# boguszjelinski/taxidispatcher

Measured on AMD Instinct MI355X. Metric: NxN assignments/sec, higher is better.
Workload: dtype int32; 1 GPU; g1 N=16384: device cost write (4N^2 B) + exact assignment, total checked == optimum; n=16384, parallelism=single GPU

## Files before the change

taxidispatcher_amd/csrc/td_assign.hip:

```cpp
#include <dlfcn.h>
#include <limits.h>
#include <stdlib.h>

#include <type_traits>

#include "td_common.h"

using namespace td;

namespace {

template <typename CT>
struct Tr;
template <>
struct Tr<uint8_t> {
    using PT = int32_t;
    static constexpr int E = 16;
    static constexpr uint32_t SENT = 0xFFu;
    static constexpr int64_t LIMIT = 254;
    static constexpr int32_t BIG = 1 << 28;
    static constexpr int32_t KMAX = INT32_MAX;
};
template <>
struct Tr<uint16_t> {
// ... 130 lines not shown
int g_defer_const = 1;
int g_shape = 1;
int g_shape_max_n = 1 << 20;
int g_narrow_price = 1;
long long g_np_plimit = NP_PLIMIT;
int g_fuse_t = 2;
int g_fuse_spec = 1;
int g_fused_rounds = 8;
int g_fuse_gen = 1;
int g_tick_rounds = 5;
int g_forest = 1;
int g_forest_min_n = 2048;
long long g_forest_w0 = 16;
long long g_forest_wx = 16;
int g_blocks = -1;
int g_blocks_min_n = 12288;
int g_zs_rounds = 4;
int g_zs_sep = 0;
int g_hop_passes = 2;
int g_hop_max_rows = HOP_FMAX;
int g_lazy_cc = 1;
int g_hop_global = 1;
int g_one_trip = 1;
int g_zs_global_rounds = 6;
int g_core = 1;
int g_core_k = 64;
int g_core_min_n = 8192;
int g_core_mode = 1;
double g_core_eps = 1.0;
int g_rand_test = 1;
int g_rand_div = 8192;
int g_rand_rounds = 48;
int g_rand_repeat = 1;
double g_rand_corr = 0.12;
int g_core_patience = 6;
int g_solver_eps = 0;
int g_eps_theta = 8;
long long g_eps0_mult = 4;
void read_tunables()
{
    static bool done = false;
    if (done) return;
    done = true;
    if (const char *e = getenv("TD_MAX_ROUNDS")) g_max_rounds = std::max(1, std::min(48, atoi(e)));
    if (const char *e = getenv("TD_TIE_EVICT")) g_tie_evict = atoi(e) != 0;
    if (const char *e = getenv("TD_LDS_ROUNDS")) g_lds_rounds = std::max(0, atoi(e));
// ... 47 lines not shown
    if (const char *e = getenv("TD_LINE")) g_line = atoi(e) != 0;
    if (const char *e = getenv("TD_LINE_MIN_N")) g_line_min_n = std::max(2, atoi(e));
    if (const char *e = getenv("TD_PSAP8_GRID")) g_psap8_grid = std::max(1, std::min(192, atoi(e)));
    if (const char *e = getenv("TD_CORE")) g_core = atoi(e) != 0;
    if (const char *e = getenv("TD_CORE_K")) g_core_k = std::max(2, std::min(200, atoi(e)));
    if (const char *e = getenv("TD_CORE_MIN_N")) g_core_min_n = std::max(256, atoi(e));
    if (const char *e = getenv("TD_CORE_MODE")) g_core_mode = atoi(e);
    if (const char *e = getenv("TD_CORE_EPS")) g_core_eps = atof(e);
    if (const char *e = getenv("TD_CORE_PATIENCE")) g_core_patience = std::max(1, atoi(e));
    if (const char *e = getenv("TD_RAND_TEST")) g_rand_test = atoi(e) != 0;
    if (const char *e = getenv("TD_RAND_DIV")) g_rand_div = std::max(1, atoi(e));
    if (const char *e = getenv("TD_RAND_ROUNDS")) g_rand_rounds = std::max(1, std::min(48, atoi(e)));
    if (const char *e = getenv("TD_RAND_CORR")) g_rand_corr = atof(e);
    if (const char *e = getenv("TD_RAND_REPEAT")) g_rand_repeat = std::max(1, atoi(e));
    if (const char *e = getenv("TD_BLOCKS")) g_blocks = std::max(-1, std::min(HOP_BMAX, atoi(e)));
    if (const char *e = getenv("TD_BLOCKS_MIN_N")) g_blocks_min_n = std::max(0, atoi(e));
    if (const char *e = getenv("TD_ZS_ROUNDS")) g_zs_rounds = std::max(0, std::min(32, atoi(e)));
    if (const char *e = getenv("TD_ZS_SEP")) g_zs_sep = atoi(e) != 0;
    if (const char *e = getenv("TD_HOP_PASSES")) g_hop_passes = std::max(0, std::min(8, atoi(e)));
    if (const char *e = getenv("TD_HOP_MAX_ROWS")) g_hop_max_rows = std::max(1, atoi(e));
    if (const char *e = getenv("TD_HOP_GLOBAL")) g_hop_global = atoi(e) != 0;
    if (const char *e = getenv("TD_ONE_TRIP")) g_one_trip = atoi(e) != 0;
    if (const char *e = getenv("TD_LAZY_CC")) g_lazy_cc = atoi(e) != 0;
    if (const char *e = getenv("TD_ZS_GLOBAL_ROUNDS")) g_zs_global_rounds = std::max(1, std::min(48, atoi(e)));
}

template <typename CT>
__device__ __forceinline__ void unpack(const uint4 &v, uint32_t *out);
template <>
__device__ __forceinline__ void unpack<uint8_t>(const uint4 &v, uint32_t *o)
{
    const uint32_t w[4] = {v.x, v.y, v.z, v.w};
#pragma unroll
    for (int k = 0; k < 4; k++) {
        o[4 * k + 0] = w[k] & 0xFFu;
        o[4 * k + 1] = (w[k] >> 8) & 0xFFu;
        o[4 * k + 2] = (w[k] >> 16) & 0xFFu;
        o[4 * k + 3] = w[k] >> 24;
    }
}
template <>
__device__ __forceinline__ void unpack<u8e>(const uint4 &v, uint32_t *o)
{
    const uint32_t w[4] = {v.x, v.y, v.z, v.w};
    const uint32_t esc = g_esc8;
#pragma unroll
// ... 144 lines not shown
__global__ __launch_bounds__(256) void k_compress_rest(int n, int nrows, int row0, int nchunks, int rpb, const int32_t *__restrict__ cost,
                                                       uint8_t *__restrict__ cc, const int32_t *__restrict__ rowmin,
                                                       const int *__restrict__ ctl)
{
    if (ctl[CTL_FLAG]) return;
    const int nq = n >> 2, qpb = rpb >> 2;
    const size_t pitch = (size_t)nchunks * 16;
    for (int row = blockIdx.x; row < nrows; row += gridDim.x) {
        const int mn = rowmin[row];
        const int q0 = ((row0 + row) / rpb) * qpb;
        const int4 *s4 = reinterpret_cast<const int4 *>(cost + (int64_t)row * n);
        uint32_t *dst = reinterpret_cast<uint32_t *>(cc + (size_t)row * pitch);
        for (int q = threadIdx.x; q < nq; q += 256) {
            if ((unsigned)(q - q0) < (unsigned)qpb) continue;
            const int4 x4 = s4[q];
            const uint32_t a = (uint32_t)(x4.x - mn), b = (uint32_t)(x4.y - mn), c = (uint32_t)(x4.z - mn), d = (uint32_t)(x4.w - mn);
            dst[q] = (a & 0xFF) | ((b & 0xFF) << 8) | ((c & 0xFF) << 16) | (d << 24);
        }
    }
}

__device__ __forceinline__ void shape_decide(int n, int *__restrict__ ctl);

template <typename CT, int VPT, int THREADS, bool BID0 = false, int LH = 0>
__global__ __launch_bounds__(THREADS) void k_compress_reg(
    int n, int nrows, int nchunks, const int32_t *__restrict__ cost, CT *__restrict__ cc, int32_t *__restrict__ rowmin, int *__restrict__ ctl,
    int *__restrict__ rconst, const long long *__restrict__ skip, unsigned long long *__restrict__ bid = nullptr, int row0 = 0,
    int *__restrict__ r2c = nullptr ,
    int probe_tickets = 0 ,
    int zs_rpb = 0 ,
    int diag_only = 0 )
{
    static_assert(!BID0 || sizeof(CT) == 1, "round 0 out of the compress pass: 1-byte cells");
    if (skip && *skip) return;
    constexpr int E = Tr<CT>::E;
    constexpr int NW = THREADS / 64;
    __shared__ int s_mn[2][NW], s_mx[2][NW];
    __shared__ int s_fp[2][BID0 ? NW : 1], s_c0[2][BID0 ? NW : 1];
    const int tid = threadIdx.x, lane = tid & 63, w = tid >> 6;
    const size_t pitch = (size_t)nchunks * E;
    const int nq = n >> 2;
    int par = 0;
    int prev_row = -1, prev_rot = 0;
    long long wmax = 0;
    auto flush_bid = [&](int slot) {
        if constexpr (BID0) {
            if (prev_row < 0 || w != 0) return;
            int fp = INT_MAX, c0 = 0;
#pragma unroll
            for (int k = 0; k < NW; k++) {
// ... 14 lines not shown
                }
#pragma unroll
                for (int o = 32; o > 0; o >>= 1) m2 = min(m2, (unsigned)__shfl_xor((int)m2, o));
            }
            if (lane == 0) {
                const int grow = row0 + prev_row;
                const int t1 = fp / E;
                int ch = t1 + prev_rot;
                if (zs_rpb) {
                    const int zcpb = zs_rpb / E;
                    if (ch >= zcpb) ch -= zcpb;
                    ch += (grow / zs_rpb) * zcpb;
                } else if (ch >= nchunks)
                    ch -= nchunks;
                const int j1 = ch * E + (fp - t1 * E);
                const unsigned long long inc = (c0 >= 2 || m2 == 255) ? 0ull : (unsigned long long)m2;
                if (inc == 0 && (grow & 15) == 0) atomicAdd(&ctl[CTL_TIED], 1);
                if (j1 < n) atomicMax(&bid[j1], (inc << ROW_BITS) | (unsigned long long)(grow + 1));
            }
        }
    };
    constexpr int VR = VPT - LH;
    extern __shared__ int4 s_rowh[];
    for (int row = blockIdx.x; row < nrows; row += gridDim.x) {
        const int4 *s4 = reinterpret_cast<const int4 *>(cost + (int64_t)row * n);
        int4 v[VPT];
#pragma unroll
        for (int k = 0; k < VPT; k++) {
            const int q = k * THREADS + tid;
#if defined(TD_NT) && (TD_NT & 2)
            if (q < nq) {
                typedef int v4i __attribute__((ext_vector_type(4)));
                const v4i t4 = __builtin_nontemporal_load(reinterpret_cast<const v4i *>(s4) + q);
                v[k] = make_int4(t4.x, t4.y, t4.z, t4.w);
            }
#else
            if (q < nq) v[k] = s4[q];
#endif
        }
        int mn = INT_MAX, mx = INT_MIN;
#pragma unroll
        for (int k = 0; k < VPT; k++) {
            const int q = k * THREADS + tid;
            if (q < nq) {
                mn = min(min(mn, v[k].x), min(v[k].y, min(v[k].z, v[k].w)));
                mx = max(max(mx, v[k].x), max(v[k].y, max(v[k].z, v[k].w)));
            }
// ... 2410 lines not shown
            using PT = typename Tr<CT>::PT;
            const int npad = nchunks * E;
            const PT padkey = (PT)(Tr<CT>::BIG << 1) | (PT)1;
            const int gi = (std::max(npad, (int)CTL_WORDS) + 255) / 256;
            const int gc = nq <= 256 * 16 ? gb : std::max(1, std::min(nrows, c.n_cu * 2));
            tickets = sv.probe ? gi + gc : 0;
            uint8_t *ob_z = nullptr;
            if (g_one_trip && zs_rpb > 0) {
                if ((rc = ensure(sv.ob, (size_t)npad + 64))) return rc;
                ob_z = (uint8_t *)sv.ob.p;
            }
            unsigned long long *fin_z = g_one_trip ? (unsigned long long *)((char *)sv.misc.p + FIN_OFF) : nullptr;
            k_init_state<PT><<<gi, 256, 0, c.stream>>>(n, npad, nrows, (PT *)sv.price.p, padkey, (int *)sv.owner.p, (int *)sv.r2c.p,
                                                       (unsigned long long *)sv.bid.p, ctl, nullptr, sv.probe, tickets, ob_z, fin_z);
            if (!fin_z) TD_HIP(hipMemsetAsync((char *)sv.misc.p + FIN_OFF, 0, 16, c.stream));
            sv.ob_clear = ob_z != nullptr;
            sv.bid0_done = true;
        }
        ProfScope ps(TD_K_COMPRESS);
        unsigned long long *bidp = (unsigned long long *)sv.bid.p;
        int *defer_r2c = sv.defer_const ? (int *)sv.r2c.p : nullptr;
        if (g_creg && vec && nq <= 256 * 16) {
            const int g2 = std::max(1, std::min(nrows, c.n_cu * g_cgrid));
#define TD_CR(VPT) k_compress_reg<CT, VPT, 256><<<g2, 256, 0, c.stream>>>(n, nrows, nchunks, sv.d_cost, cc, rm, ctl, rcs, sv.skip)
            if (nq <= 256) { TD_CR(1); }
            else if (nq <= 512) { TD_CR(2); }
            else if (nq <= 1024) { TD_CR(4); }
            else if (nq <= 2048) { TD_CR(8); }
            else if (bid0_kernel) {
                if constexpr (sizeof(CT) == 1) {
                    static const int shape = getenv("TD_BID0_SHAPE") ? atoi(getenv("TD_BID0_SHAPE")) : 0;
                    if (shape == 1)
                        k_compress_reg<CT, 4, 1024, true><<<gb, 1024, 0, c.stream>>>(n, nrows, nchunks, sv.d_cost, cc, rm, ctl, rcs, sv.skip, bidp,
                                                                                    sv.row0, defer_r2c, tickets, zs_rpb, diag);
                    else
                        k_compress_reg<CT, 8, 512, true><<<gb, 512, 0, c.stream>>>(n, nrows, nchunks, sv.d_cost, cc, rm, ctl, rcs, sv.skip, bidp,
                                                                                   sv.row0, defer_r2c, tickets, zs_rpb, diag);
                    sv.zs_done = zs_rpb > 0;
                    sv.cc_partial = diag != 0;
                    sv.cc_rpb = zs_rpb;
                }
            } else {
                static const int cshape = getenv("TD_CREG_SHAPE") ? atoi(getenv("TD_CREG_SHAPE")) : 0;
                if (cshape == 1)
                    k_compress_reg<CT, 8, 512><<<gb, 512, 0, c.stream>>>(n, nrows, nchunks, sv.d_cost, cc, rm, ctl, rcs, sv.skip);
                else if (cshape == 2)
                    k_compress_reg<CT, 4, 1024><<<gb, 1024, 0, c.stream>>>(n, nrows, nchunks, sv.d_cost, cc, rm, ctl, rcs, sv.skip);
                else { TD_CR(16); }
            }
#undef TD_CR
        } else if (g_creg && vec && nq <= 1024 * 16) {
            const int g4 = std::max(1, std::min(nrows, c.n_cu * 2));
            static const int clds = getenv("TD_CLDS") ? atoi(getenv("TD_CLDS")) : 0;
            if (bid0_kernel) {
                if constexpr (sizeof(CT) == 1)
                {
                    if (clds == 8) {
                        const int shm = 8 * 1024 * 16;
                        (void)hipFuncSetAttribute((const void *)k_compress_reg<CT, 16, 1024, true, 8>, hipFuncAttributeMaxDynamicSharedMemorySize, shm);
                        k_compress_reg<CT, 16, 1024, true, 8><<<g4, 1024, shm, c.stream>>>(n, nrows, nchunks, sv.d_cost, cc, rm, ctl, rcs, sv.skip, bidp,
                                                                                          sv.row0, defer_r2c, tickets, zs_rpb, diag);
                    } else if (clds == 4) {
                        const int shm = 4 * 1024 * 16;
                        (void)hipFuncSetAttribute((const void *)k_compress_reg<CT, 16, 1024, true, 4>, hipFuncAttributeMaxDynamicSharedMemorySize, shm);
                        k_compress_reg<CT, 16, 1024, true, 4><<<g4, 1024, shm, c.stream>>>(n, nrows, nchunks, sv.d_cost, cc, rm, ctl, rcs, sv.skip, bidp,
                                                                                          sv.row0, defer_r2c, tickets, zs_rpb, diag);
                    } else
                        k_compress_reg<CT, 16, 1024, true><<<g4, 1024, 0, c.stream>>>(n, nrows, nchunks, sv.d_cost, cc, rm, ctl, rcs, sv.skip, bidp,
                                                                                      sv.row0, defer_r2c, tickets, zs_rpb, diag);
                    sv.zs_done = zs_rpb > 0;
                    sv.cc_partial = diag != 0;
                    sv.cc_rpb = zs_rpb;
                }
            } else
                k_compress_reg<CT, 16, 1024><<<g4, 1024, 0, c.stream>>>(n, nrows, nchunks, sv.d_cost, cc, rm, ctl, rcs, sv.skip);
        } else if (vec)
            k_compress<CT, true><<<grid, 256, 0, c.stream>>>(n, nrows, nchunks, sv.d_cost, cc, rm, ctl, rcs, sv.skip);
        else
            k_compress<CT, false><<<grid, 256, 0, c.stream>>>(n, nrows, nchunks, sv.d_cost, cc, rm, ctl, rcs, sv.skip);
    }
    TD_HIP(hipGetLastError());
    if (speculate) {
        *fits = true;
        sv.nconst = -1;
    } else {
        TD_HIP(hipMemcpyAsync(c.pinned, ctl, CTL_ALL * sizeof(int), hipMemcpyDeviceToHost, c.stream));
        TD_HIP(hipStreamSynchronize(c.stream));
        *fits = (((int *)c.pinned)[CTL_FLAG] == 0);
        sv.nconst = ((int *)c.pinned)[CTL_NCONST];
        sv.range_seen = (int64_t)(((const unsigned long long *)((int *)c.pinned + CTL_RSEEN))[0]);
        if (!*fits) c.stats[6] = (int64_t)(((const unsigned long long *)((int *)c.pinned + CTL_RANGE))[0]);
    }
    if (*fits) {
        sv.bpc = IsNP<CT>::value ? 5 : (int)sizeof(CT);
        sv.nchunks = nchunks;
        sv.npad = nchunks * E;
    }
    return TD_OK;
// ... 79 lines not shown
    *range = (int64_t)(((const unsigned long long *)(h + CTL_RANGE))[0]);
    *fits = h[CTL_FLAG] == 0 && *range <= (int64_t)Tr<uint32_t>::LIMIT && *range >= 0;
    sv.nconst = h[CTL_NCONST];
    if (*fits) {
        sv.nchunks = nchunks;
        sv.npad = npad;
    }
    return TD_OK;
}

int sv_complete_cc(Solver &sv)
{
    if (!sv.cc_partial) return TD_OK;
    Ctx &c = ctx();
    ProfScope ps(TD_K_COMPRESS);
    k_compress_rest<<<std::max(1, std::min(sv.nrows, c.n_cu * 8)), 256, 0, c.stream>>>(sv.n, sv.nrows, sv.row0, sv.nchunks, sv.cc_rpb, sv.d_cost,
                                                                                      (uint8_t *)sv.cc.p, (const int32_t *)sv.rowmin.p,
                                                                                      (const int *)sv.misc.p);
    TD_HIP(hipGetLastError());
    sv.cc_partial = false;
    return TD_OK;
}

template <typename CT>
int sv_hop_t(Solver &sv, int rpb, int ncols_blk, int col_lo, int nb, bool window_zero, uint8_t *ob, bool raw = false, bool gate = false)
{
    Ctx &c = ctx();
    using PT = typename Tr<CT>::PT;
    int rc;
    if ((rc = ensure(sv.esc, sizeof(unsigned long long) * 2 * (size_t)std::max(sv.nrows, 1)))) return rc;
    if ((rc = ensure(sv.hop, sizeof(HopCtl)))) return rc;
    if ((rc = ensure(sv.hoptab, sizeof(int) * (size_t)nb * HOP_FMAX * HOP_FMAX))) return rc;
    HopCtl *hc = (HopCtl *)sv.hop.p;
    int *frl = (int *)sv.list.p, *fcl = (int *)sv.pred.p;
    const int *ctl = (const int *)sv.misc.p;
    if (gate && nb != 1) return fail(TD_EINTERNAL, "a gated two-hop pass takes one block");
    k_hop_lists<<<nb, 1024, 0, c.stream>>>(rpb, ncols_blk, col_lo, (const int *)sv.r2c.p, (const int *)sv.owner.p, frl, fcl, hc, ctl,
                                           gate ? g_hop_max_rows : 0);
    if (raw) {
        if (!sv.d_cost || sv.n % 4) return fail(TD_EINVAL, "two-hop pass on the int32 matrix: no matrix, or n %% 4 != 0");
        k_hop_esc<CT, true><<<(sv.nrows + 3) / 4, 256, 0, c.stream>>>(sv.nrows, sv.n / 4, rpb, ncols_blk, col_lo, g_hop_max_rows,
                                                                      (const CT *)sv.d_cost, (const PT *)sv.price.p, (const int *)sv.r2c.p, fcl,
                                                                      hc, (unsigned long long *)sv.esc.p, ctl, (const int32_t *)sv.rowmin.p);
        k_hop_table<CT, true><<<nb * HOP_FMAX, 256, 0, c.stream>>>(sv.n, sv.nrows, sv.row0, sv.n / 4, rpb, ncols_blk, col_lo, g_hop_max_rows,
                                                                   window_zero ? 1 : 0, (const CT *)sv.d_cost, (const PT *)sv.price.p,
                                                                   (const int *)sv.owner.p, frl, hc, (const unsigned long long *)sv.esc.p,
                                                                   (int *)sv.hoptab.p, ctl, (const int32_t *)sv.rowmin.p);
    } else {
    k_hop_esc<CT><<<(sv.nrows + 3) / 4, 256, 0, c.stream>>>(sv.nrows, sv.nchunks, rpb, ncols_blk, col_lo, g_hop_max_rows, (const CT *)sv.cc.p,
                                                            (const PT *)sv.price.p, (const int *)sv.r2c.p, fcl, hc,
                                                            (unsigned long long *)sv.esc.p, ctl);
    k_hop_table<CT><<<nb * HOP_FMAX, 256, 0, c.stream>>>(sv.n, sv.nrows, sv.row0, sv.nchunks, rpb, ncols_blk, col_lo, g_hop_max_rows,
                                                         window_zero ? 1 : 0, (const CT *)sv.cc.p, (const PT *)sv.price.p,
                                                         (const int *)sv.owner.p, frl, hc, (const unsigned long long *)sv.esc.p,
                                                         (int *)sv.hoptab.p, ctl);
    }
    k_hop_match<PT><<<nb, HOP_FMAX, sizeof(uint32_t) * (size_t)((rpb + 31) / 32), c.stream>>>(
        sv.nrows, sv.row0, rpb, ncols_blk, col_lo, g_hop_max_rows, (PT *)sv.price.p, (int *)sv.owner.p, (int *)sv.r2c.p, ob, frl, fcl, hc,
        (const int *)sv.hoptab.p, (int *)sv.misc.p);
    TD_HIP(hipGetLastError());
    return TD_OK;
}

template <typename CT>
int sv_begin_t(Solver &sv);

int sv_phase_a(Solver &sv, int hop_passes)
{
    Ctx &c = ctx();
    const int n = sv.n, nrows = sv.nrows;
    const int rpb = n / sv.zs_V, nb = nrows / rpb;
    const int col_lo = (sv.row0 / rpb) * rpb, col_hi = col_lo + nb * rpb;
    int rc;
    if ((rc = ensure(sv.ob, (size_t)sv.npad + 64))) return rc;
    if (!sv.ob_clear) TD_HIP(hipMemsetAsync(sv.ob.p, 0, (size_t)sv.npad, c.stream));
    sv.ob_clear = false;
    ProfScope ps(TD_K_BID);
    int *ctl = (int *)sv.misc.p;
    const int ga = (col_hi - col_lo + 255) / 256;
    unsigned long long *bid = (unsigned long long *)sv.bid.p;
    auto assign = [&]() {
        k_zs_assign<<<ga, 256, 0, c.stream>>>(col_lo, col_hi, nrows, sv.row0, bid, (int32_t *)sv.price.p, (int *)sv.owner.p, (int *)sv.r2c.p,
                                              (uint8_t *)sv.ob.p, ctl);
    };
    if (sv.zs_round0) {
        if (!sv.began && (rc = sv_begin_t<uint8_t>(sv))) return rc;
        k_zs_bid<<<std::min(nrows, c.n_cu * 16), 256, 0, c.stream>>>(nrows, sv.row0, sv.nchunks, rpb, (const uint8_t *)sv.cc.p,
                                                                     (const uint8_t *)sv.ob.p, (const int *)sv.r2c.p, bid, ctl, 0, 0);
        sv.zs_round0 = false;
    }
    assign();
    for (int r = 1; r <= g_zs_rounds; r++) {
        k_zs_bid<<<std::min(nrows, c.n_cu * 16), 256, 0, c.stream>>>(nrows, sv.row0, sv.nchunks, rpb, (const uint8_t *)sv.cc.p,
                                                                     (const uint8_t *)sv.ob.p, (const int *)sv.r2c.p, bid, ctl, r, g_tie_evict);
        assign();
    }
    TD_HIP(hipGetLastError());
    for (int p = 0; p < hop_passes; p++)
        if ((rc = sv_hop_t<uint8_t>(sv, rpb, rpb, col_lo, nb, true, (uint8_t *)sv.ob.p))) return rc;
    if (getenv("TD_DEBUG") && hop_passes > 0) {
        HopCtl h;
        TD_HIP(hipMemcpyAsync(&h, sv.hop.p, sizeof(h), hipMemcpyDeviceToHost, c.stream));
        TD_HIP(hipStreamSynchronize(c.stream));
        fprintf(stderr, "[td] phase A: %d blocks of %d rows, %d local rounds; free rows / columns per block before the last two-hop pass:", nb, rpb, g_zs_rounds);
        for (int b = 0; b < nb; b++) fprintf(stderr, " %d/%d", h.nfr[b], h.nfc[b]);
        fprintf(stderr, " | matched %d, left %d\n", h.matched, h.left);
    }
    sv.zs_done = false;
    sv.bid0_done = false;
    sv.state_ready = true;
    return TD_OK;
}

template <typename CT>
int sv_begin_t(Solver &sv)
{
    Ctx &c = ctx();
    using PT = typename Tr<CT>::PT;
    const PT padkey = (PT)(Tr<CT>::BIG << 1) | (PT)1;
    k_init_state<PT><<<(std::max(sv.npad, (int)CTL_WORDS) + 255) / 256, 256, 0, c.stream>>>(
        sv.n, sv.npad, sv.nrows, (PT *)sv.price.p, padkey, (int *)sv.owner.p, (int *)sv.r2c.p,
        (unsigned long long *)sv.bid.p, (int *)sv.misc.p, sv.defer_const ? (const int *)sv.rconst.p : nullptr, sv.probe, 0, nullptr,
// ... 874 lines not shown
        auto rounds = [&](bool first) -> int {
            for (int r = 0; r < round_cap; r++) {
                rc = TD_OK;
                if (!(r == 0 && first && sv.bid0_done)) TD_DISPATCH(sv, sv_bid_t, sv, r, (unsigned long long *)sv.bid.p);
                if (rc) return rc;
                TD_DISPATCH(sv, sv_apply_t, sv, r, (unsigned long long *)sv.bid.p);
                if (rc) return rc;
            }
            return TD_OK;
        };
        bool random_like = false;
        auto warm = [&](int bits) -> int {
            const int keep = g_warm_bits;
            g_warm_bits = bits;
            if (bpc == 2) rc = sv_warm_t<uint16_t>(sv, known_range, &warm_rounds, &random_like);
            else if (bpc == 5) rc = sv_warm_t<u32n>(sv, known_range, &warm_rounds, &random_like);
            else rc = sv_warm_t<uint32_t>(sv, known_range, &warm_rounds, &random_like);
            g_warm_bits = keep;
            return rc;
        };
        bool all_placed = false;
        if (sv.zs_done) {
            const int passes_a = g_hop_passes;
            if ((rc = sv_phase_a(sv, passes_a))) return rc;
            if (passes_a > 0 && g_one_trip && !transposed && !sv.gen) {
                if (g_hop_global && (rc = sv_hop_t<uint8_t>(sv, n, n, 0, 1, true, nullptr, sv.cc_partial, true))) return rc;
                const bool dev_out = is_device_ptr(row_to_col);
                r2c_in_pinned = !dev_out && (size_t)R2C_PIN_OFF + sizeof(int32_t) * (size_t)n <= c.pinned_cap;
                int *r2c_out = dev_out ? row_to_col : (r2c_in_pinned ? (int *)((char *)c.pinned + R2C_PIN_OFF) : nullptr);
                if ((rc = sv_end_gated(sv, dual_bound != nullptr, r2c_out))) return rc;
                TD_HIP(hipStreamSynchronize(c.stream));
                const char *rec = (const char *)c.pinned + REC_OFF;
                const int left = ((const int *)rec)[REC_LEFT / sizeof(int)], rflag = ((const int *)rec)[CTL_FLAG];
                if (left < 0) return fail(TD_EINTERNAL, "the end-of-solve record was not written");
                if (getenv("TD_DEBUG")) fprintf(stderr, "[td] one trip: %d rows free after the two-hop passes, flag %d\n", left, rflag);
                if (left == 0 && rflag == 0) {
                    int flag = 0;
                    if ((rc = sv_readback_parse(sv, rec, &tot, &dual, max_rounds, &flag))) return rc;
                    c.stats[1] = 0;
                    c.stats[6] = 0;
                    r2c_on_device = dev_out;
                    solved = true;
                    break;
                }
                r2c_in_pinned = false;
                round_cap = std::min(max_rounds, g_zs_global_rounds);
            } else if (passes_a > 0) {
                int *pin = (int *)c.pinned;
                auto read_left = [&]() -> int {
// ... 781 lines not shown
```

taxidispatcher_amd/csrc/td_blocks.h:

```cpp


struct HopCtl {
    int nfr[HOP_BMAX], nfc[HOP_BMAX];
    int left;
    int matched;
    int pad[2];
};

__device__ __forceinline__ uint32_t zs_zero_bytes(uint32_t w)
{
    return ~(((w & 0x7F7F7F7Fu) + 0x7F7F7F7Fu) | w | 0x7F7F7F7Fu);
}

__global__ __launch_bounds__(256) void k_zs_bid(int nrows, int row0, int nchunks, int rpb, const uint8_t *__restrict__ cc,
                                                const uint8_t *__restrict__ ob, const int *__restrict__ r2c,
                                                unsigned long long *__restrict__ bid, const int *__restrict__ ctl, int round,
                                                int tie_evict)
{
    __shared__ int s_best[4];
    if (ctl[CTL_FLAG]) return;
    const int tid = threadIdx.x, lane = tid & 63, w = tid >> 6;
    const int cpb = rpb >> 4;
    const size_t pitch = (size_t)nchunks * 16;
    for (int lrow = blockIdx.x; lrow < nrows; lrow += gridDim.x) {
        if (r2c[lrow] != -1) continue;
        const int row = row0 + lrow;
        const int c0 = (row / rpb) * cpb;
        const uint32_t hsh = ((uint32_t)row + 1u) * 0x9E3779B1u + (uint32_t)round * 0x85EBCA6Bu;
        const int rot = (int)(((uint64_t)(hsh ^ (hsh >> 15)) * (uint64_t)cpb) >> 32);
// ... 15 lines not shown
                const int cand = (zf ? 0 : (1 << 24)) | (t * 16 + k * 4 + (__builtin_ctz(pick) >> 3));
                best = min(best, cand);
            }
        }
#pragma unroll
        for (int o = 32; o > 0; o >>= 1) best = min(best, __shfl_xor(best, o));
        if (lane == 0) s_best[w] = best;
        __syncthreads();
        if (tid == 0) {
            best = min(min(s_best[0], s_best[1]), min(s_best[2], s_best[3]));
            if (best != INT_MAX) {
                const bool owned = (best >> 24) != 0;
                const int pos = best & 0xFFFFFF;
                int ch = (pos >> 4) + rot;
                if (ch >= cpb) ch -= cpb;
                const int j = (c0 + ch) * 16 + (pos & 15);
                if (!owned || tie_evict) atomicMax(&bid[j], (unsigned long long)(row + 1));
            }
        }
        __syncthreads();
    }
}

__global__ __launch_bounds__(256) void k_zs_assign(int col_lo, int col_hi, int nrows, int row0, unsigned long long *__restrict__ bid,
                                                   int32_t *__restrict__ pk, int *__restrict__ owner, int *__restrict__ r2c,
                                                   uint8_t *__restrict__ ob, const int *__restrict__ ctl)
{
    if (ctl[CTL_FLAG]) return;
    const int j = col_lo + blockIdx.x * blockDim.x + threadIdx.x;
    if (j >= col_hi) return;
    const unsigned long long k = bid[j];
    if (!k) return;
    const int row = (int)(k & ((1ull << ROW_BITS) - 1)) - 1;
    const int old = owner[j];
    if (old >= row0 && old < row0 + nrows) r2c[old - row0] = -1;
    owner[j] = row;
    if (row >= row0 && row < row0 + nrows) r2c[row - row0] = j;
    pk[j] = 1;
    ob[j] = 1;
    bid[j] = 0ull;
}

__global__ __launch_bounds__(1024) void k_hop_lists(int rpb, int ncols_blk, int col_lo, const int *__restrict__ r2c,
                                                    const int *__restrict__ owner, int *__restrict__ frl, int *__restrict__ fcl,
                                                    HopCtl *__restrict__ hc, const int *__restrict__ ctl, int gate_max = 0)
{
    if (ctl[CTL_FLAG]) return;
    const int lb = blockIdx.x;
    if (gate_max > 0) {
        __shared__ int s_go;
        if (threadIdx.x == 0) {
            const int left = hc->left;
            s_go = left > 0 && left <= gate_max;
        }
        __syncthreads();
        if (!s_go) {
            if (threadIdx.x == 0) hc->nfr[lb] = 0, hc->nfc[lb] = 0;
            return;
        }
    }
    const int nfr = build_free_list(rpb, r2c + (size_t)lb * rpb, frl + (size_t)lb * rpb, -1);
    const int nfc = build_free_list(ncols_blk, owner + col_lo + (size_t)lb * ncols_blk, fcl + (size_t)lb * ncols_blk, -1);
    if (threadIdx.x == 0) {
// ... 164 lines not shown
            const int r = owner[s_cand[k]];
            if (r < row0 || r >= row0 + nrows) continue;
            if ((r - row0) / rpb != lb) continue;
            unsigned long long m0 = esc[(size_t)(r - row0) * 2], m1 = esc[(size_t)(r - row0) * 2 + 1];
            while (m0) {
                const int b = __builtin_ctzll(m0);
                m0 &= m0 - 1;
                atomicMin(&s_tab[b], r);
            }
            while (m1) {
                const int b = 64 + __builtin_ctzll(m1);
                m1 &= m1 - 1;
                atomicMin(&s_tab[b], r);
            }
        }
        __syncthreads();
        if (tid == 0) s_ncand = 0;
        __syncthreads();
    }
    if (tid < HOP_FMAX) tab[((size_t)lb * HOP_FMAX + a) * HOP_FMAX + tid] = s_tab[tid] == INT_MAX ? -1 : s_tab[tid];
}

template <typename PT>
__global__ __launch_bounds__(HOP_FMAX) void k_hop_match(int nrows, int row0, int rpb, int ncols_blk, int col_lo, int max_rows,
                                                        PT *__restrict__ pk, int *__restrict__ owner, int *__restrict__ r2c,
                                                        uint8_t *__restrict__ ob, const int *__restrict__ frl,
                                                        const int *__restrict__ fcl, HopCtl *__restrict__ hc,
                                                        const int *__restrict__ tab, int *__restrict__ ctl)
{
    extern __shared__ uint32_t s_usedr[];
    __shared__ int s_usedc[HOP_FMAX];
    __shared__ int s_key[2][2];
    if (ctl[CTL_FLAG]) return;
    const int lb = blockIdx.x;
    const int nfr = hc->nfr[lb];
    const int tid = threadIdx.x, lane = tid & 63, w = tid >> 6;
    if (nfr == 0) return;
    if (nfr > max_rows) {
        if (tid == 0) atomicAdd(&hc->left, nfr);
        return;
    }
    const int na = min(nfr, HOP_FMAX), nc = min(hc->nfc[lb], HOP_FMAX);
    for (int k = tid; k < (rpb + 31) / 32; k += HOP_FMAX) s_usedr[k] = 0u;
    s_usedc[tid] = 0;
    __syncthreads();
    const int *fr = frl + (size_t)lb * rpb, *fc = fcl + (size_t)lb * ncols_blk;
    const int blk_row0 = row0 + lb * rpb;
    const int my_fc = tid < nc ? fc[tid] : 0;
    int done = 0;
    int r_nx = tid < nc ? tab[((size_t)lb * HOP_FMAX + 0) * HOP_FMAX + tid] : -1;
    int i_nx = blk_row0 + fr[0];
    for (int a = 0; a < na; a++) {
        const int r = r_nx, i_g = i_nx;
        if (a + 1 < na) {
            r_nx = tid < nc ? tab[((size_t)lb * HOP_FMAX + a + 1) * HOP_FMAX + tid] : -1;
            i_nx = blk_row0 + fr[a + 1];
// ... 17 lines not shown
        best = min(s_key[a & 1][0], s_key[a & 1][1]);
        if (best != INT_MAX && key == best) {
            const int rl = r - row0, il = i_g - row0;
            const int j = r2c[rl], jp = col_lo + lb * ncols_blk + my_fc;
            r2c[il] = j;
            owner[j] = i_g;
            r2c[rl] = jp;
            owner[jp] = r;
            pk[jp] = pk[jp] | (PT)1;
            if (ob) ob[jp] = 1;
            s_usedc[tid] = 1;
            const int rb = r - blk_row0;
            atomicOr(&s_usedr[rb >> 5], 1u << (rb & 31));
        }
        if (best != INT_MAX) done++;
        __syncthreads();
    }
    if (tid == 0) {
        atomicAdd(&hc->left, nfr - done);
        atomicAdd(&hc->matched, done);
    }
}

__global__ void k_zs_owned_bits(int n, const int *__restrict__ owner, int32_t *__restrict__ pk)
{
    const int j = blockIdx.x * blockDim.x + threadIdx.x;
    if (j < n) pk[j] = (pk[j] & ~1) | (owner[j] >= 0 ? 1 : 0);
}
```

Baseline: 27.49 million assignments/s.

## Fold hop free-list construction into assign and match kernels via last-block tickets

Builds the per-block free row and column lists for the two-hop pass inside the final k_zs_assign launch and at the tail of k_hop_match. The last block to finish, found with an atomic ticket plus release/acquire fences, builds the lists, so the separate k_hop_lists launches can be skipped. This removes several small kernel launches and their serialization on the stream, at the cost of extra fence and atomic-ticket overhead and single-block list building at the tail. It also adds an optional row-order parameter to the compress kernel, which defaults to the original order.

```diff
diff --git a/taxidispatcher_amd/csrc/td_assign.hip b/taxidispatcher_amd/csrc/td_assign.hip
--- a/taxidispatcher_amd/csrc/td_assign.hip
+++ b/taxidispatcher_amd/csrc/td_assign.hip
@@ -176,6 +176,8 @@
 int g_lazy_cc = 1;
 int g_hop_global = 1;
 int g_one_trip = 1;
+int g_compress_order = 0;
+int g_hop_fold = 1;
 int g_zs_global_rounds = 6;
 int g_core = 1;
 int g_core_k = 64;
@@ -269,6 +271,8 @@
     if (const char *e = getenv("TD_HOP_GLOBAL")) g_hop_global = atoi(e) != 0;
     if (const char *e = getenv("TD_ONE_TRIP")) g_one_trip = atoi(e) != 0;
     if (const char *e = getenv("TD_LAZY_CC")) g_lazy_cc = atoi(e) != 0;
+    if (const char *e = getenv("TD_COMPRESS_ORDER")) g_compress_order = std::max(0, std::min(2, atoi(e)));
+    if (const char *e = getenv("TD_HOP_FOLD")) g_hop_fold = atoi(e) != 0;
     if (const char *e = getenv("TD_ZS_GLOBAL_ROUNDS")) g_zs_global_rounds = std::max(1, std::min(48, atoi(e)));
 }
 
@@ -459,10 +463,26 @@
 
 __device__ __forceinline__ void shape_decide(int n, int *__restrict__ ctl);
 
+__device__ __forceinline__ int compress_row(int order, int it, int nrows)
+{
+    const int b = blockIdx.x, g = gridDim.x;
+    if (order == 2 && g >= 8 && nrows >= 8) {
+        const int x = b & 7;
+        const int lo = (int)(((long long)x * nrows) >> 3), hi = (int)(((long long)(x + 1) * nrows) >> 3);
+        const int wx = (g - x + 7) >> 3;
+        const long long i = (long long)(b >> 3) + (long long)it * wx;
+        return i < hi - lo ? hi - 1 - (int)i : -1;
+    }
+    const long long i = (long long)b + (long long)it * g;
+    if (i >= nrows) return -1;
+    return order == 0 ? (int)i : nrows - 1 - (int)i;
+}
+
 template <typename CT, int VPT, int THREADS, bool BID0 = false, int LH = 0>
 __global__ __launch_bounds__(THREADS) void k_compress_reg(
     int n, int nrows, int nchunks, const int32_t *__restrict__ cost, CT *__restrict__ cc, int32_t *__restrict__ rowmin, int *__restrict__ ctl,
-    int *__restrict__ rconst, const long long *__restrict__ skip, unsigned long long *__restrict__ bid = nullptr, int row0 = 0,
+    int *__restrict__ rconst, const long long *__restrict__ skip, int order ,
+    unsigned long long *__restrict__ bid = nullptr, int row0 = 0,
     int *__restrict__ r2c = nullptr ,
     int probe_tickets = 0 ,
     int zs_rpb = 0 ,
@@ -523,7 +543,7 @@
     };
     constexpr int VR = VPT - LH;
     extern __shared__ int4 s_rowh[];
-    for (int row = blockIdx.x; row < nrows; row += gridDim.x) {
+    for (int it = 0, row; (row = compress_row(order, it, nrows)) >= 0; it++) {
         const int4 *s4 = reinterpret_cast<const int4 *>(cost + (int64_t)row * n);
         int4 v[VPT];
 #pragma unroll
@@ -2980,7 +3000,7 @@
         int *defer_r2c = sv.defer_const ? (int *)sv.r2c.p : nullptr;
         if (g_creg && vec && nq <= 256 * 16) {
             const int g2 = std::max(1, std::min(nrows, c.n_cu * g_cgrid));
-#define TD_CR(VPT) k_compress_reg<CT, VPT, 256><<<g2, 256, 0, c.stream>>>(n, nrows, nchunks, sv.d_cost, cc, rm, ctl, rcs, sv.skip)
+#define TD_CR(VPT) k_compress_reg<CT, VPT, 256><<<g2, 256, 0, c.stream>>>(n, nrows, nchunks, sv.d_cost, cc, rm, ctl, rcs, sv.skip, g_compress_order)
             if (nq <= 256) { TD_CR(1); }
             else if (nq <= 512) { TD_CR(2); }
             else if (nq <= 1024) { TD_CR(4); }
@@ -2989,10 +3009,10 @@
                 if constexpr (sizeof(CT) == 1) {
                     static const int shape = getenv("TD_BID0_SHAPE") ? atoi(getenv("TD_BID0_SHAPE")) : 0;
                     if (shape == 1)
-                        k_compress_reg<CT, 4, 1024, true><<<gb, 1024, 0, c.stream>>>(n, nrows, nchunks, sv.d_cost, cc, rm, ctl, rcs, sv.skip, bidp,
+                        k_compress_reg<CT, 4, 1024, true><<<gb, 1024, 0, c.stream>>>(n, nrows, nchunks, sv.d_cost, cc, rm, ctl, rcs, sv.skip, g_compress_order, bidp,
                                                                                     sv.row0, defer_r2c, tickets, zs_rpb, diag);
                     else
-                        k_compress_reg<CT, 8, 512, true><<<gb, 512, 0, c.stream>>>(n, nrows, nchunks, sv.d_cost, cc, rm, ctl, rcs, sv.skip, bidp,
+                        k_compress_reg<CT, 8, 512, true><<<gb, 512, 0, c.stream>>>(n, nrows, nchunks, sv.d_cost, cc, rm, ctl, rcs, sv.skip, g_compress_order, bidp,
                                                                                    sv.row0, defer_r2c, tickets, zs_rpb, diag);
                     sv.zs_done = zs_rpb > 0;
                     sv.cc_partial = diag != 0;
@@ -3001,9 +3021,9 @@
             } else {
                 static const int cshape = getenv("TD_CREG_SHAPE") ? atoi(getenv("TD_CREG_SHAPE")) : 0;
                 if (cshape == 1)
-                    k_compress_reg<CT, 8, 512><<<gb, 512, 0, c.stream>>>(n, nrows, nchunks, sv.d_cost, cc, rm, ctl, rcs, sv.skip);
+                    k_compress_reg<CT, 8, 512><<<gb, 512, 0, c.stream>>>(n, nrows, nchunks, sv.d_cost, cc, rm, ctl, rcs, sv.skip, g_compress_order);
                 else if (cshape == 2)
-                    k_compress_reg<CT, 4, 1024><<<gb, 1024, 0, c.stream>>>(n, nrows, nchunks, sv.d_cost, cc, rm, ctl, rcs, sv.skip);
+                    k_compress_reg<CT, 4, 1024><<<gb, 1024, 0, c.stream>>>(n, nrows, nchunks, sv.d_cost, cc, rm, ctl, rcs, sv.skip, g_compress_order);
                 else { TD_CR(16); }
             }
 #undef TD_CR
@@ -3016,22 +3036,22 @@
                     if (clds == 8) {
                         const int shm = 8 * 1024 * 16;
                         (void)hipFuncSetAttribute((const void *)k_compress_reg<CT, 16, 1024, true, 8>, hipFuncAttributeMaxDynamicSharedMemorySize, shm);
-                        k_compress_reg<CT, 16, 1024, true, 8><<<g4, 1024, shm, c.stream>>>(n, nrows, nchunks, sv.d_cost, cc, rm, ctl, rcs, sv.skip, bidp,
+                        k_compress_reg<CT, 16, 1024, true, 8><<<g4, 1024, shm, c.stream>>>(n, nrows, nchunks, sv.d_cost, cc, rm, ctl, rcs, sv.skip, g_compress_order, bidp,
                                                                                           sv.row0, defer_r2c, tickets, zs_rpb, diag);
                     } else if (clds == 4) {
                         const int shm = 4 * 1024 * 16;
                         (void)hipFuncSetAttribute((const void *)k_compress_reg<CT, 16, 1024, true, 4>, hipFuncAttributeMaxDynamicSharedMemorySize, shm);
-                        k_compress_reg<CT, 16, 1024, true, 4><<<g4, 1024, shm, c.stream>>>(n, nrows, nchunks, sv.d_cost, cc, rm, ctl, rcs, sv.skip, bidp,
+                        k_compress_reg<CT, 16, 1024, true, 4><<<g4, 1024, shm, c.stream>>>(n, nrows, nchunks, sv.d_cost, cc, rm, ctl, rcs, sv.skip, g_compress_order, bidp,
                                                                                           sv.row0, defer_r2c, tickets, zs_rpb, diag);
                     } else
-                        k_compress_reg<CT, 16, 1024, true><<<g4, 1024, 0, c.stream>>>(n, nrows, nchunks, sv.d_cost, cc, rm, ctl, rcs, sv.skip, bidp,
+                        k_compress_reg<CT, 16, 1024, true><<<g4, 1024, 0, c.stream>>>(n, nrows, nchunks, sv.d_cost, cc, rm, ctl, rcs, sv.skip, g_compress_order, bidp,
                                                                                       sv.row0, defer_r2c, tickets, zs_rpb, diag);
                     sv.zs_done = zs_rpb > 0;
                     sv.cc_partial = diag != 0;
                     sv.cc_rpb = zs_rpb;
                 }
             } else
-                k_compress_reg<CT, 16, 1024><<<g4, 1024, 0, c.stream>>>(n, nrows, nchunks, sv.d_cost, cc, rm, ctl, rcs, sv.skip);
+                k_compress_reg<CT, 16, 1024><<<g4, 1024, 0, c.stream>>>(n, nrows, nchunks, sv.d_cost, cc, rm, ctl, rcs, sv.skip, g_compress_order);
         } else if (vec)
             k_compress<CT, true><<<grid, 256, 0, c.stream>>>(n, nrows, nchunks, sv.d_cost, cc, rm, ctl, rcs, sv.skip);
         else
@@ -3157,21 +3177,32 @@
     return TD_OK;
 }
 
+int ensure_hop(Solver &sv)
+{
+    const bool fresh = !sv.hop.p || sv.hop.cap < sizeof(HopCtl);
+    int rc;
+    if ((rc = ensure(sv.hop, sizeof(HopCtl)))) return rc;
+    if (fresh) TD_HIP(hipMemsetAsync(sv.hop.p, 0, sizeof(HopCtl), ctx().stream));
+    return TD_OK;
+}
+
 template <typename CT>
-int sv_hop_t(Solver &sv, int rpb, int ncols_blk, int col_lo, int nb, bool window_zero, uint8_t *ob, bool raw = false, bool gate = false)
+int sv_hop_t(Solver &sv, int rpb, int ncols_blk, int col_lo, int nb, bool window_zero, uint8_t *ob, bool raw = false, bool gate = false,
+             bool lists_ready = false, int next = 0, int gate_n = 0)
 {
     Ctx &c = ctx();
     using PT = typename Tr<CT>::PT;
     int rc;
     if ((rc = ensure(sv.esc, sizeof(unsigned long long) * 2 * (size_t)std::max(sv.nrows, 1)))) return rc;
-    if ((rc = ensure(sv.hop, sizeof(HopCtl)))) return rc;
+    if ((rc = ensure_hop(sv))) return rc;
     if ((rc = ensure(sv.hoptab, sizeof(int) * (size_t)nb * HOP_FMAX * HOP_FMAX))) return rc;
     HopCtl *hc = (HopCtl *)sv.hop.p;
     int *frl = (int *)sv.list.p, *fcl = (int *)sv.pred.p;
     const int *ctl = (const int *)sv.misc.p;
     if (gate && nb != 1) return fail(TD_EINTERNAL, "a gated two-hop pass takes one block");
-    k_hop_lists<<<nb, 1024, 0, c.stream>>>(rpb, ncols_blk, col_lo, (const int *)sv.r2c.p, (const int *)sv.owner.p, frl, fcl, hc, ctl,
-                                           gate ? g_hop_max_rows : 0);
+    if (!lists_ready)
+        k_hop_lists<<<nb, 1024, 0, c.stream>>>(rpb, ncols_blk, col_lo, (const int *)sv.r2c.p, (const int *)sv.owner.p, frl, fcl, hc, ctl,
+                                               gate ? g_hop_max_rows : 0);
     if (raw) {
         if (!sv.d_cost || sv.n % 4) return fail(TD_EINVAL, "two-hop pass on the int32 matrix: no matrix, or n %% 4 != 0");
         k_hop_esc<CT, true><<<(sv.nrows + 3) / 4, 256, 0, c.stream>>>(sv.nrows, sv.n / 4, rpb, ncols_blk, col_lo, g_hop_max_rows,
@@ -3192,7 +3223,7 @@
     }
     k_hop_match<PT><<<nb, HOP_FMAX, sizeof(uint32_t) * (size_t)((rpb + 31) / 32), c.stream>>>(
         sv.nrows, sv.row0, rpb, ncols_blk, col_lo, g_hop_max_rows, (PT *)sv.price.p, (int *)sv.owner.p, (int *)sv.r2c.p, ob, frl, fcl, hc,
-        (const int *)sv.hoptab.p, (int *)sv.misc.p);
+        (const int *)sv.hoptab.p, (int *)sv.misc.p, next, gate_n, g_hop_max_rows);
     TD_HIP(hipGetLastError());
     return TD_OK;
 }
@@ -3200,7 +3231,7 @@
 template <typename CT>
 int sv_begin_t(Solver &sv);
 
-int sv_phase_a(Solver &sv, int hop_passes)
+int sv_phase_a(Solver &sv, int hop_passes, bool gate_after = false)
 {
     Ctx &c = ctx();
     const int n = sv.n, nrows = sv.nrows;
@@ -3214,9 +3245,12 @@
     int *ctl = (int *)sv.misc.p;
     const int ga = (col_hi - col_lo + 255) / 256;
     unsigned long long *bid = (unsigned long long *)sv.bid.p;
-    auto assign = [&]() {
+    const bool fold = g_hop_fold && hop_passes > 0;
+    if (fold && (rc = ensure_hop(sv))) return rc;
+    auto assign = [&](bool last = false) {
         k_zs_assign<<<ga, 256, 0, c.stream>>>(col_lo, col_hi, nrows, sv.row0, bid, (int32_t *)sv.price.p, (int *)sv.owner.p, (int *)sv.r2c.p,
-                                              (uint8_t *)sv.ob.p, ctl);
+                                              (uint8_t *)sv.ob.p, ctl, fold && last ? rpb : 0, (int *)sv.list.p, (int *)sv.pred.p,
+                                              (HopCtl *)sv.hop.p);
     };
     if (sv.zs_round0) {
         if (!sv.began && (rc = sv_begin_t<uint8_t>(sv))) return rc;
@@ -3224,15 +3258,17 @@
                                                                      (const uint8_t *)sv.ob.p, (const int *)sv.r2c.p, bid, ctl, 0, 0);
         sv.zs_round0 = false;
     }
-    assign();
+    assign(g_zs_rounds == 0);
     for (int r = 1; r <= g_zs_rounds; r++) {
         k_zs_bid<<<std::min(nrows, c.n_cu * 16), 256, 0, c.stream>>>(nrows, sv.row0, sv.nchunks, rpb, (const uint8_t *)sv.cc.p,
                                                                      (const uint8_t *)sv.ob.p, (const int *)sv.r2c.p, bid, ctl, r, g_tie_evict);
-        assign();
+        assign(r == g_zs_rounds);
     }
     TD_HIP(hipGetLastError());
-    for (int p = 0; p < hop_passes; p++)
-        if ((rc = sv_hop_t<uint8_t>(sv, rpb, rpb, col_lo, nb, true, (uint8_t *)sv.ob.p))) return rc;
+    for (int p = 0; p < hop_passes; p++) {
+        const int next = !fold ? 0 : (p + 1 < hop_passes ? 1 : (gate_after ? 2 : 0));
+        if ((rc = sv_hop_t<uint8_t>(sv, rpb, rpb, col_lo, nb, true, (uint8_t *)sv.ob.p, false, false, fold, next, n))) return rc;
+    }
     if (getenv("TD_DEBUG") && hop_passes > 0) {
         HopCtl h;
         TD_HIP(hipMemcpyAsync(&h, sv.hop.p, sizeof(h), hipMemcpyDeviceToHost, c.stream));
@@ -4153,9 +4189,11 @@
         bool all_placed = false;
         if (sv.zs_done) {
             const int passes_a = g_hop_passes;
-            if ((rc = sv_phase_a(sv, passes_a))) return rc;
-            if (passes_a > 0 && g_one_trip && !transposed && !sv.gen) {
-                if (g_hop_global && (rc = sv_hop_t<uint8_t>(sv, n, n, 0, 1, true, nullptr, sv.cc_partial, true))) return rc;
+            const bool one_trip = passes_a > 0 && g_one_trip && !transposed && !sv.gen;
+            const bool fold_gate = one_trip && g_hop_global && g_hop_fold;
+            if ((rc = sv_phase_a(sv, passes_a, fold_gate))) return rc;
+            if (one_trip) {
+                if (g_hop_global && (rc = sv_hop_t<uint8_t>(sv, n, n, 0, 1, true, nullptr, sv.cc_partial, true, fold_gate))) return rc;
                 const bool dev_out = is_device_ptr(row_to_col);
                 r2c_in_pinned = !dev_out && (size_t)R2C_PIN_OFF + sizeof(int32_t) * (size_t)n <= c.pinned_cap;
                 int *r2c_out = dev_out ? row_to_col : (r2c_in_pinned ? (int *)((char *)c.pinned + R2C_PIN_OFF) : nullptr);
diff --git a/taxidispatcher_amd/csrc/td_blocks.h b/taxidispatcher_amd/csrc/td_blocks.h
--- a/taxidispatcher_amd/csrc/td_blocks.h
+++ b/taxidispatcher_amd/csrc/td_blocks.h
@@ -4,7 +4,9 @@
     int nfr[HOP_BMAX], nfc[HOP_BMAX];
     int left;
     int matched;
-    int pad[2];
+    int tk_match;
+    int pad;
+    int tk_blk[HOP_BMAX];
 };
 
 __device__ __forceinline__ uint32_t zs_zero_bytes(uint32_t w)
@@ -66,23 +68,100 @@
     }
 }
 
+__device__ __forceinline__ int build_free_list_coh(int n, const int *src, int *__restrict__ list, int want)
+{
+    __shared__ int s_flc_w[16];
+    const int tid = threadIdx.x, lane = tid & 63, w = tid >> 6, nw = blockDim.x >> 6;
+    const int seg = (((n + nw - 1) / nw) + 63) & ~63;
+    const int lo = min(n, w * seg), hi = min(n, lo + seg);
+    int cnt = 0;
+#pragma unroll 4
+    for (int r = lo; r < hi; r += 64) {
+        const int i = r + lane;
+        const int x = i < hi ? __hip_atomic_load(src + i, __ATOMIC_RELAXED, __HIP_MEMORY_SCOPE_AGENT) : ~want;
+        cnt += (int)__popcll(__ballot(x == want));
+    }
+    if (lane == 0) s_flc_w[w] = cnt;
+    __syncthreads();
+    int pos = 0, tot = 0;
+    for (int k = 0; k < nw; k++) {
+        const int v = s_flc_w[k];
+        pos += k < w ? v : 0;
+        tot += v;
+    }
+    if (cnt) {
+        for (int r = lo; r < hi; r += 64) {
+            const int i = r + lane;
+            const int x = i < hi ? __hip_atomic_load(src + i, __ATOMIC_RELAXED, __HIP_MEMORY_SCOPE_AGENT) : ~want;
+            const unsigned long long m = __ballot(x == want);
+            if (x == want) list[pos + (int)__popcll(m & ((1ull << lane) - 1ull))] = i;
+            pos += (int)__popcll(m);
+        }
+    }
+    __syncthreads();
+    return tot;
+}
+
+__device__ __forceinline__ bool fold_ticket(int *ticket, int expect, bool acquire)
+{
+    __shared__ int s_ft_last;
+    asm volatile("s_waitcnt vmcnt(0)" ::: "memory");
+    __syncthreads();
+    if (threadIdx.x == 0) {
+        __builtin_amdgcn_fence(__ATOMIC_RELEASE, "agent");
+        asm volatile("s_waitcnt vmcnt(0)" ::: "memory");
+        const bool last = atomicAdd(ticket, 1) == expect - 1;
+        if (last && acquire) {
+            __builtin_amdgcn_fence(__ATOMIC_ACQUIRE, "agent");
+            asm volatile("s_waitcnt vmcnt(0)" ::: "memory");
+        }
+        s_ft_last = last ? 1 : 0;
+    }
+    __syncthreads();
+    const bool last = s_ft_last != 0;
+    __syncthreads();
+    return last;
+}
+
+__device__ __forceinline__ void zs_fold_lists(int col_lo, int col_hi, int rpb, const int *r2c, const int *owner, int *__restrict__ frl,
+                                              int *__restrict__ fcl, HopCtl *__restrict__ hc)
+{
+    const int T = blockDim.x;
+    const int c0 = blockIdx.x * T, c1 = min(c0 + T, col_hi - col_lo) - 1;
+    for (int lb = c0 / rpb; lb <= c1 / rpb; lb++) {
+        const int first = (lb * rpb) / T, last = ((lb + 1) * rpb - 1) / T;
+        if (!fold_ticket(&hc->tk_blk[lb], last - first + 1, true)) continue;
+        const int nfr = build_free_list_coh(rpb, r2c + (size_t)lb * rpb, frl + (size_t)lb * rpb, -1);
+        const int nfc = build_free_list_coh(rpb, owner + col_lo + (size_t)lb * rpb, fcl + (size_t)lb * rpb, -1);
+        if (threadIdx.x == 0) {
+            hc->nfr[lb] = nfr;
+            hc->nfc[lb] = nfc;
+            if (lb == 0) hc->left = 0, hc->matched = 0;
+            hc->tk_blk[lb] = 0;
+        }
+    }
+}
+
 __global__ __launch_bounds__(256) void k_zs_assign(int col_lo, int col_hi, int nrows, int row0, unsigned long long *__restrict__ bid,
-                                                   int32_t *__restrict__ pk, int *__restrict__ owner, int *__restrict__ r2c,
-                                                   uint8_t *__restrict__ ob, const int *__restrict__ ctl)
+                                                   int32_t *__restrict__ pk, int *owner, int *r2c,
+                                                   uint8_t *__restrict__ ob, const int *__restrict__ ctl, int fold_rpb = 0,
+                                                   int *__restrict__ frl = nullptr, int *__restrict__ fcl = nullptr,
+                                                   HopCtl *__restrict__ hc = nullptr)
 {
     if (ctl[CTL_FLAG]) return;
     const int j = col_lo + blockIdx.x * blockDim.x + threadIdx.x;
-    if (j >= col_hi) return;
-    const unsigned long long k = bid[j];
-    if (!k) return;
-    const int row = (int)(k & ((1ull << ROW_BITS) - 1)) - 1;
-    const int old = owner[j];
-    if (old >= row0 && old < row0 + nrows) r2c[old - row0] = -1;
-    owner[j] = row;
-    if (row >= row0 && row < row0 + nrows) r2c[row - row0] = j;
-    pk[j] = 1;
-    ob[j] = 1;
-    bid[j] = 0ull;
+    const unsigned long long k = j < col_hi ? bid[j] : 0ull;
+    if (k) {
+        const int row = (int)(k & ((1ull << ROW_BITS) - 1)) - 1;
+        const int old = owner[j];
+        if (old >= row0 && old < row0 + nrows) r2c[old - row0] = -1;
+        owner[j] = row;
+        if (row >= row0 && row < row0 + nrows) r2c[row - row0] = j;
+        pk[j] = 1;
+        ob[j] = 1;
+        bid[j] = 0ull;
+    }
+    if (fold_rpb > 0) zs_fold_lists(col_lo, col_hi, fold_rpb, r2c, owner, frl, fcl, hc);
 }
 
 __global__ __launch_bounds__(1024) void k_hop_lists(int rpb, int ncols_blk, int col_lo, const int *__restrict__ r2c,
@@ -293,16 +372,14 @@
 }
 
 template <typename PT>
-__global__ __launch_bounds__(HOP_FMAX) void k_hop_match(int nrows, int row0, int rpb, int ncols_blk, int col_lo, int max_rows,
-                                                        PT *__restrict__ pk, int *__restrict__ owner, int *__restrict__ r2c,
-                                                        uint8_t *__restrict__ ob, const int *__restrict__ frl,
-                                                        const int *__restrict__ fcl, HopCtl *__restrict__ hc,
-                                                        const int *__restrict__ tab, int *__restrict__ ctl)
+__device__ __forceinline__ void hop_match_block(int nrows, int row0, int rpb, int ncols_blk, int col_lo, int max_rows, PT *__restrict__ pk,
+                                                int *__restrict__ owner, int *__restrict__ r2c, uint8_t *__restrict__ ob,
+                                                const int *__restrict__ frl, const int *__restrict__ fcl, HopCtl *__restrict__ hc,
+                                                const int *__restrict__ tab)
 {
     extern __shared__ uint32_t s_usedr[];
     __shared__ int s_usedc[HOP_FMAX];
     __shared__ int s_key[2][2];
-    if (ctl[CTL_FLAG]) return;
     const int lb = blockIdx.x;
     const int nfr = hc->nfr[lb];
     const int tid = threadIdx.x, lane = tid & 63, w = tid >> 6;
@@ -366,6 +443,56 @@
     }
 }
 
+__device__ __forceinline__ void hop_fold_next(int next, int rpb, int ncols_blk, int col_lo, int gate_n, int gate_max, const int *r2c,
+                                              const int *owner, int *__restrict__ frl, int *__restrict__ fcl, HopCtl *__restrict__ hc)
+{
+    __shared__ int s_hf_go;
+    const int lb = blockIdx.x, tid = threadIdx.x;
+    if (next == 1) {
+        asm volatile("s_waitcnt vmcnt(0)" ::: "memory");
+        __syncthreads();
+        const int nfr = build_free_list_coh(rpb, r2c + (size_t)lb * rpb, frl + (size_t)lb * rpb, -1);
+        const int nfc = build_free_list_coh(ncols_blk, owner + col_lo + (size_t)lb * ncols_blk, fcl + (size_t)lb * ncols_blk, -1);
+        if (tid == 0) hc->nfr[lb] = nfr, hc->nfc[lb] = nfc;
+    }
+    if (!fold_ticket(&hc->tk_match, (int)gridDim.x, next == 2)) return;
+    if (next == 1) {
+        if (tid == 0) {
+            __hip_atomic_store(&hc->left, 0, __ATOMIC_RELAXED, __HIP_MEMORY_SCOPE_AGENT);
+            __hip_atomic_store(&hc->matched, 0, __ATOMIC_RELAXED, __HIP_MEMORY_SCOPE_AGENT);
+            hc->tk_match = 0;
+        }
+        return;
+    }
+    if (tid == 0) {
+        const int left = __hip_atomic_load(&hc->left, __ATOMIC_RELAXED, __HIP_MEMORY_SCOPE_AGENT);
+        s_hf_go = left > 0 && left <= gate_max;
+    }
+    __syncthreads();
+    if (!s_hf_go) {
+        if (tid == 0) hc->nfr[0] = 0, hc->nfc[0] = 0, hc->tk_match = 0;
+        return;
+    }
+    const int nfr = build_free_list_coh(gate_n, r2c, frl, -1);
+    const int nfc = build_free_list_coh(gate_n, owner, fcl, -1);
+    if (tid == 0) {
+        hc->nfr[0] = nfr, hc->nfc[0] = nfc, hc->tk_match = 0;
+        __hip_atomic_store(&hc->left, 0, __ATOMIC_RELAXED, __HIP_MEMORY_SCOPE_AGENT);
+        __hip_atomic_store(&hc->matched, 0, __ATOMIC_RELAXED, __HIP_MEMORY_SCOPE_AGENT);
+    }
+}
+
+template <typename PT>
+__global__ __launch_bounds__(HOP_FMAX) void k_hop_match(int nrows, int row0, int rpb, int ncols_blk, int col_lo, int max_rows, PT *pk,
+                                                        int *owner, int *r2c, uint8_t *ob, int *frl, int *fcl, HopCtl *hc,
+                                                        const int *__restrict__ tab, int *__restrict__ ctl, int next = 0, int gate_n = 0,
+                                                        int gate_max = 0)
+{
+    if (ctl[CTL_FLAG]) return;
+    hop_match_block<PT>(nrows, row0, rpb, ncols_blk, col_lo, max_rows, pk, owner, r2c, ob, frl, fcl, hc, tab);
+    if (next) hop_fold_next(next, rpb, ncols_blk, col_lo, gate_n, gate_max, r2c, owner, frl, fcl, hc);
+}
+
 __global__ void k_zs_owned_bits(int n, const int *__restrict__ owner, int32_t *__restrict__ pk)
 {
     const int j = blockIdx.x * blockDim.x + threadIdx.x;
```

Result: slower. 23.06 million assignments/s (-16.1%).
